# rushi-the-neural-arch/PyTorch-DistributedTraining

Hardware: AMD Instinct MI355X
Metric: tokens/sec GPT-2-1.3B FSDP (whole node) (higher is better)
Workload: dtype bf16; 1 GPU; model=gpt2-1.3b, global_batch=96, seq_len=1024, parallelism=fsdp1, micro_batch_per_gpu=96, params=1313722368, hip_graph=False, optimizer=fused AdamW + global-norm clip

## Files before the change

### csrc/kernels/gemm.hip

```cpp
#include "common.h"
#include "gelu.h"
#include "reduce.h"
#include <stdlib.h>
#include <type_traits>

using namespace pdt;

namespace {

typedef __bf16 bf16x8_t __attribute__((ext_vector_type(8)));
typedef short v4i16 __attribute__((ext_vector_type(4)));
typedef int v4i __attribute__((ext_vector_type(4)));
typedef __attribute__((address_space(3))) v4i16 lds_v4i16;
typedef __attribute__((address_space(3))) u16x8 lds_u16x8;
typedef __attribute__((address_space(3))) void lds_void;
typedef __attribute__((address_space(3))) const char lds_cchar;

constexpr int TM = 256, TN = 256, KB = 64, NTH = 256;
constexpr int OPB = TM * KB * 2;
constexpr int STB = 2 * OPB;
constexpr int PIECES = OPB / (NTH * 16);

enum { L_NT = 0, L_TT = 1 };
enum { E_PLAIN = 0, E_BIAS = 1, E_GELU = 2, E_DGELU = 3, E_F32 = 4 };
// ... 306 lines not shown
    if constexpr (EPI == E_DGELU) {
#pragma unroll
      for (int j = 0; j < 8; ++j)
#pragma unroll
        for (int r = 0; r < 4; ++r) {
          float v = cs[j][r];
          v += __shfl_xor(v, 1);
          v += __shfl_xor(v, 2);
          v += __shfl_xor(v, 4);
          v += __shfl_xor(v, 8);
          cs[j][r] = v;
        }
      __syncthreads();
      float* red = reinterpret_cast<float*>(smem);
      if ((lane & 15) == 0) {
#pragma unroll
        for (int j = 0; j < 8; ++j)
#pragma unroll
          for (int r = 0; r < 4; ++r) red[wr * 256 + 128 * wc + 16 * j + 4 * (lane >> 4) + r] = cs[j][r];
      }
      __syncthreads();
      p.ws[(int64_t)tm * p.N + n0 + tid] = red[tid] + red[256 + tid];
    }
  }
  }
}

}
#include "gemm_kloop.inc"
namespace {

constexpr int RING = 2 * STB;
constexpr int STAGE_BYTES = 32768;
constexpr int SMEM3 = RING + STAGE_BYTES;

template <int I, int N, class F>
__device__ __forceinline__ void sfor(F&& f) {
  if constexpr (I < N) {
    f(std::integral_constant<int, I>{});
    sfor<I + 1, N>(f);
  }
}

template <int K>
__device__ __forceinline__ f32x4 acc_tile() {
  float x, y, z, w;
  asm volatile("v_accvgpr_read_b32 %0, a%c4\n\tv_accvgpr_read_b32 %1, a%c5\n\t"
               "v_accvgpr_read_b32 %2, a%c6\n\tv_accvgpr_read_b32 %3, a%c7"
               : "=v"(x), "=v"(y), "=v"(z), "=v"(w)
               : "i"(4 * K), "i"(4 * K + 1), "i"(4 * K + 2), "i"(4 * K + 3));
  return f32x4{x, y, z, w};
}

__device__ __forceinline__ uint32_t stg_off(int q, int col) {
  return (uint32_t)(q * 512 + ((((col >> 3) ^ q) & 15) | ((col >> 3) & 16)) * 16 + (col & 7) * 2);
}
__device__ __forceinline__ int stg_row(int r, int q) { return 128 * (q >> 5) + 32 * r + (q & 31); }
__device__ __forceinline__ void stg_read(const char* img, u16x8 (&buf)[8], int w, int lane) {
#pragma unroll
  for (int it = 0; it < 8; ++it) {
    const int q = 16 * w + 2 * it + (lane >> 5), c16 = lane & 31;
    buf[it] = *reinterpret_cast<const u16x8*>(img + q * 512 + ((c16 ^ (q & 15)) & 15 | (c16 & 16)) * 16);
  }
}
typedef unsigned int u32x4 __attribute__((ext_vector_type(4)));
__device__ __forceinline__ __amdgpu_buffer_rsrc_t tile_rsrc(const bf16_t* base, int64_t ldc, int m0, int n0) {
  return __builtin_amdgcn_make_buffer_rsrc((void*)(base + (int64_t)m0 * ldc + n0), (short)0,
                                           (int)((255 * ldc + 256) * 2), 0x00020000);
}
__device__ __forceinline__ uint32_t stg_voff(int64_t ldc, int w, int lane) {
  return (uint32_t)(128 * (w >> 1) + 16 * (w & 1) + (lane >> 5)) * ((uint32_t)ldc * 2u) + (uint32_t)(lane & 31) * 16u;
}
__device__ __forceinline__ float row16_sum(float v) {
  v += __int_as_float(__builtin_amdgcn_update_dpp(0, __float_as_int(v), 0xB1, 0xF, 0xF, false));
  v += __int_as_float(__builtin_amdgcn_update_dpp(0, __float_as_int(v), 0x4E, 0xF, 0xF, false));
  v += __int_as_float(__builtin_amdgcn_update_dpp(0, __float_as_int(v), 0x141, 0xF, 0xF, false));
  v += __int_as_float(__builtin_amdgcn_update_dpp(0, __float_as_int(v), 0x140, 0xF, 0xF, false));
  return v;
}
__device__ __forceinline__ void stg_write_out(const u16x8 (&buf)[8], __amdgpu_buffer_rsrc_t rs, uint32_t vo,
                                              uint32_t ldc2, int r) {
#pragma unroll
  for (int it = 0; it < 8; ++it)
    __builtin_amdgcn_raw_buffer_store_b128(__builtin_bit_cast(u32x4, buf[it]), rs, (int)vo,
                                           (int)((32 * r + 2 * it) * ldc2), 0);
}
__device__ __forceinline__ void stg_fetch(u16x8 (&t)[8], __amdgpu_buffer_rsrc_t rs, uint32_t vo, uint32_t ldc2, int r) {
#pragma unroll
  for (int it = 0; it < 8; ++it)
    t[it] = __builtin_bit_cast(u16x8, __builtin_amdgcn_raw_buffer_load_b128(rs, (int)vo,
                                                                            (int)((32 * r + 2 * it) * ldc2), 0));
}
__device__ __forceinline__ void stg_put(char* img, const u16x8 (&t)[8], int w, int lane) {
#pragma unroll
  for (int it = 0; it < 8; ++it) {
    const int q = 16 * w + 2 * it + (lane >> 5), c16 = lane & 31;
    *reinterpret_cast<u16x8*>(img + q * 512 + ((c16 ^ (q & 15)) & 15 | (c16 & 16)) * 16) = t[it];
  }
}
__device__ __forceinline__ void stg_dma_round0(const bf16_t* src, int64_t ldc, int m0, int n0, uint32_t img_lds,
                                               int w, int lane) {
  const uint64_t base = (uint64_t)(uintptr_t)(src + (int64_t)m0 * ldc + n0);
  v4i rsrc;
  rsrc[0] = (int)(uint32_t)base;
  rsrc[1] = (int)((base >> 32) & 0xffff);
  rsrc[2] = (int)(uint32_t)((255 * ldc + 256) * 2);
  rsrc[3] = 0x00020000;
  const int hi = lane >> 5, p = lane & 31;
  const uint32_t row0 = (uint32_t)(128 * (w >> 1) + 16 * (w & 1));
  const uint32_t ldc2 = (uint32_t)ldc * 2u;
  uint32_t vo[8], so[8];
#pragma unroll
  for (int i = 0; i < 8; ++i) {
    const uint32_t c16 = (uint32_t)(((p ^ (2 * i + hi)) & 15) | (p & 16));
    vo[i] = (uint32_t)hi * ldc2 + c16 * 16u;
    so[i] = __builtin_amdgcn_readfirstlane((row0 + 2 * i) * ldc2);
  }
  const uint32_t m = __builtin_amdgcn_readfirstlane(img_lds + 16 * w * 512);
  asm volatile(
      "s_mov_b32 m0, %[m]\n\ts_nop 0\n\tbuffer_load_dwordx4 %[v0], %[rs], %[s0] offen lds\n\t"
      "s_add_u32 m0, m0, 1024\n\ts_nop 0\n\tbuffer_load_dwordx4 %[v1], %[rs], %[s1] offen lds\n\t"
      "s_add_u32 m0, m0, 1024\n\ts_nop 0\n\tbuffer_load_dwordx4 %[v2], %[rs], %[s2] offen lds\n\t"
      "s_add_u32 m0, m0, 1024\n\ts_nop 0\n\tbuffer_load_dwordx4 %[v3], %[rs], %[s3] offen lds\n\t"
      "s_add_u32 m0, m0, 1024\n\ts_nop 0\n\tbuffer_load_dwordx4 %[v4], %[rs], %[s4] offen lds\n\t"
      "s_add_u32 m0, m0, 1024\n\ts_nop 0\n\tbuffer_load_dwordx4 %[v5], %[rs], %[s5] offen lds\n\t"
      "s_add_u32 m0, m0, 1024\n\ts_nop 0\n\tbuffer_load_dwordx4 %[v6], %[rs], %[s6] offen lds\n\t"
      "s_add_u32 m0, m0, 1024\n\ts_nop 0\n\tbuffer_load_dwordx4 %[v7], %[rs], %[s7] offen lds"
      :
      : [m] "s"(m), [rs] "s"(rsrc), [v0] "v"(vo[0]), [v1] "v"(vo[1]), [v2] "v"(vo[2]), [v3] "v"(vo[3]),
        [v4] "v"(vo[4]), [v5] "v"(vo[5]), [v6] "v"(vo[6]), [v7] "v"(vo[7]), [s0] "s"(so[0]), [s1] "s"(so[1]),
        [s2] "s"(so[2]), [s3] "s"(so[3]), [s4] "s"(so[4]), [s5] "s"(so[5]), [s6] "s"(so[6]), [s7] "s"(so[7])
      : "memory", "scc");
}

__device__ __forceinline__ int item_tid(int wv) {
  int l;
  asm volatile("v_mbcnt_lo_u32_b32 %0, -1, 0\n\tv_mbcnt_hi_u32_b32 %0, -1, %0" : "=v"(l));
  return wv * 64 + l;
}
__device__ __forceinline__ int opaque_s(int x) {
  asm volatile("" : "+s"(x));
  return x;
}

__device__ __forceinline__ v4i scalar_rsrc(const void* base, uint32_t nbytes) {
  const uint64_t a = (uint64_t)(uintptr_t)base;
  v4i r;
  r[0] = (int)(uint32_t)a; r[1] = (int)((a >> 32) & 0xffff); r[2] = (int)nbytes; r[3] = 0x00020000;
  return r;
}
__device__ __forceinline__ void preload_bias(u16x4 (&b)[8], const bf16_t* bias, int n0, int lcol) {
  const v4i rs = scalar_rsrc(bias + n0, 512);
  const uint32_t vo = (uint32_t)lcol * 2u;
  asm volatile("buffer_load_dwordx2 %0, %8, %9, 0 offen offset:0\n\t"
               "buffer_load_dwordx2 %1, %8, %9, 0 offen offset:32\n\t"
               "buffer_load_dwordx2 %2, %8, %9, 0 offen offset:64\n\t"
               "buffer_load_dwordx2 %3, %8, %9, 0 offen offset:96\n\t"
               "buffer_load_dwordx2 %4, %8, %9, 0 offen offset:128\n\t"
               "buffer_load_dwordx2 %5, %8, %9, 0 offen offset:160\n\t"
               "buffer_load_dwordx2 %6, %8, %9, 0 offen offset:192\n\t"
               "buffer_load_dwordx2 %7, %8, %9, 0 offen offset:224"
               : "=&v"(b[0]), "=&v"(b[1]), "=&v"(b[2]), "=&v"(b[3]), "=&v"(b[4]), "=&v"(b[5]), "=&v"(b[6]),
                 "=&v"(b[7])
               : "v"(vo), "s"(rs)
               : "memory");
}
__device__ __forceinline__ void preload_round1(u16x8 (&t)[8], const bf16_t* src, int64_t ldc, int m0, int n0,
                                               uint32_t vo) {
  const v4i rs = scalar_rsrc(src + (int64_t)m0 * ldc + n0, (uint32_t)((255 * ldc + 256) * 2));
  const uint32_t l2 = (uint32_t)ldc * 2u;
  asm volatile("buffer_load_dwordx4 %0, %8, %9, %10 offen\n\t"
               "buffer_load_dwordx4 %1, %8, %9, %11 offen\n\t"
               "buffer_load_dwordx4 %2, %8, %9, %12 offen\n\t"
               "buffer_load_dwordx4 %3, %8, %9, %13 offen\n\t"
               "buffer_load_dwordx4 %4, %8, %9, %14 offen\n\t"
               "buffer_load_dwordx4 %5, %8, %9, %15 offen\n\t"
               "buffer_load_dwordx4 %6, %8, %9, %16 offen\n\t"
               "buffer_load_dwordx4 %7, %8, %9, %17 offen"
               : "=&v"(t[0]), "=&v"(t[1]), "=&v"(t[2]), "=&v"(t[3]), "=&v"(t[4]), "=&v"(t[5]), "=&v"(t[6]),
                 "=&v"(t[7])
               : "v"(vo), "s"(rs), "s"(32 * l2), "s"(34 * l2), "s"(36 * l2), "s"(38 * l2), "s"(40 * l2),
                 "s"(42 * l2), "s"(44 * l2), "s"(46 * l2)
               : "memory");
}
template <class V, int N>
__device__ __forceinline__ void settle(V (&x)[N]) {
#pragma unroll
  for (int i = 0; i < N; ++i) asm volatile("" : "+v"(x[i]));
}

template <int LAYOUT>
struct ItemOps {
  int tm, tn, m0, n0, split, T;
  uint32_t alo, ahi, blo, bhi;
  __device__ __forceinline__ void init(const GemmArgs& p, int item, int ntiles) {
    split = item / ntiles;
    tile_of(p, item - split * ntiles, ntiles, tm, tn);
    m0 = tm * TM; n0 = tn * TN;
    const int kbeg = split * p.k_per_split;
    T = min(p.K - kbeg, p.k_per_split) / KB;
    uint64_t a0, b0;
    if (LAYOUT == L_NT) {
      a0 = (uint64_t)(uintptr_t)p.A + ((uint64_t)m0 * p.lda + kbeg) * 2;
      b0 = (uint64_t)(uintptr_t)p.B + ((uint64_t)n0 * p.ldb + kbeg) * 2;
    } else {
      a0 = (uint64_t)(uintptr_t)p.A + ((uint64_t)kbeg * p.lda + m0) * 2;
      b0 = (uint64_t)(uintptr_t)p.B + ((uint64_t)kbeg * p.ldb + n0) * 2;
    }
    alo = (uint32_t)a0; ahi = (uint32_t)(a0 >> 32) & 0xffffu;
    blo = (uint32_t)b0; bhi = (uint32_t)(b0 >> 32) & 0xffffu;
  }
  __device__ __forceinline__ void skip2(uint64_t astep, uint64_t bstep) { skipn(2 * astep, 2 * bstep); }
  __device__ __forceinline__ void skip1(uint64_t astep, uint64_t bstep) { skipn(astep, bstep); }
  __device__ __forceinline__ void skipn(uint64_t da, uint64_t dbb) {
    const uint64_t a = (((uint64_t)ahi << 32) | alo) + da, b = (((uint64_t)bhi << 32) | blo) + dbb;
    alo = (uint32_t)a; ahi = (uint32_t)(a >> 32) & 0xffffu;
    blo = (uint32_t)b; bhi = (uint32_t)(b >> 32) & 0xffffu;
  }
};

__device__ __forceinline__ uint64_t stamp() {
  uint64_t t;
  asm volatile("s_memtime %0\n\ts_waitcnt lgkmcnt(0)" : "=s"(t) : : "memory");
  return t;
}

template <int LAYOUT, int EPI, int DIAG = 0, bool P3 = false>
__global__ __launch_bounds__(NTH, 1) void gemm_asm_kernel(GemmArgs p) {
  __shared__ __attribute__((aligned(16))) char smem[SMEM3];
  const uint32_t lds_addr = (uint32_t)(uintptr_t)(lds_void*)smem;
  const int tid = threadIdx.x, w = tid >> 6, lane = tid & 63;
  const int wr = w >> 1, wc = w & 1;
  const int wv = __builtin_amdgcn_readfirstlane(w);
  const int ntiles = (p.M / TM) * (p.N / TN);
  const int splits = (p.K + p.k_per_split - 1) / p.k_per_split;
  const int nall = ntiles * splits;

  uint64_t astep, bstep;
  uint32_t abytes, bbytes, rsa, rsb;
  int32_t db;
  if (LAYOUT == L_NT) {
    astep = bstep = KB * 2;
    abytes = (uint32_t)((TM - 1) * p.lda * 2 + KB * 2);
    bbytes = (uint32_t)((TN - 1) * p.ldb * 2 + KB * 2);
    rsa = (uint32_t)(32 * p.lda * 2);
    rsb = (uint32_t)(32 * p.ldb * 2);
    db = OPB + 16384 * (wc - wr);
  } else {
    astep = (uint64_t)KB * p.lda * 2;
    bstep = (uint64_t)KB * p.ldb * 2;
    abytes = (uint32_t)((KB - 1) * p.lda * 2 + TM * 2);
    bbytes = (uint32_t)((KB - 1) * p.ldb * 2 + TN * 2);
    rsa = (uint32_t)(8 * p.lda * 2);
    rsb = (uint32_t)(8 * p.ldb * 2);
    db = OPB + 256 * (wc - wr);
  }
  auto lane_ops = [&](int t, uint32_t& voa0, uint32_t& voa1, uint32_t& vob0, uint32_t& vob1, uint32_t& rd0,
                      uint32_t& rd1) {
    const int lw = t >> 6, ll = t & 63, lwr = lw >> 1;
    if (LAYOUT == L_NT) {
      const int row = 8 * lw + (ll >> 3);
      const int c = (ll & 7) ^ ((row >> 1) & 7);
      voa0 = voa1 = (uint32_t)(row * p.lda * 2 + c * 16);
      vob0 = vob1 = (uint32_t)(row * p.ldb * 2 + c * 16);
      const int x = ll & 15, g = ll >> 4, h = (x >> 1) & 7;
      rd0 = lds_addr + 16384 * lwr + (uint32_t)(x * 128 + 16 * (g ^ h));
      rd1 = lds_addr + 16384 * lwr + (uint32_t)(x * 128 + 16 * ((4 + g) ^ h));
    } else {
      const int r0 = 2 * lw + (ll >> 5);
      voa0 = (uint32_t)(r0 * p.lda * 2 + ((ll & 31) ^ tt_f(r0)) * 16);
      voa1 = (uint32_t)(r0 * p.lda * 2 + ((ll & 31) ^ tt_f(r0 + 8)) * 16);
      vob0 = (uint32_t)(r0 * p.ldb * 2 + ((ll & 31) ^ tt_f(r0)) * 16);
      vob1 = (uint32_t)(r0 * p.ldb * 2 + ((ll & 31) ^ tt_f(r0 + 8)) * 16);
      const int g = ll >> 4, q = (ll >> 2) & 3, pp = ll & 3;
      rd0 = lds_addr + 256 * lwr + (uint32_t)((8 * g + q) * 512 + 16 * (pp >> 1) + 8 * (pp & 1));
      rd1 = (uint32_t)tt_f(8 * g + q);
    }
  };
  const uint32_t m0b = __builtin_amdgcn_readfirstlane(lds_addr + w * 1024);
  const int dbs = __builtin_amdgcn_readfirstlane(db);
  const uint32_t asl = (uint32_t)astep, ash = (uint32_t)(astep >> 32);
  const uint32_t bsl = (uint32_t)bstep, bsh = (uint32_t)(bstep >> 32);
  constexpr int NST = EPI == E_F32 ? 64 : EPI == E_GELU ? 64 + 8 : EPI == E_DGELU ? 32 + 1 + 8 + 8 : EPI == E_BIAS ? 40 : 32;
  constexpr int WNX = 16 + NST < 63 ? 16 + NST : 63;
  char* const img = smem + RING;

#define PDT_KLOOP_CLOBBERS                                                                                      \
  "memory", "scc", "s80", "s81", "s82", "s83", "s84", "s85", "s86", "s87", "s88", "s89", "s90", "s91",         \
  "v64", "v65", "v66", "v67", "v68", "v69", "v70", "v71", "v72", "v73", "v74", "v75", "v76", "v77", "v78",     \
  "v79", "v80", "v81", "v82", "v83", "v84", "v85", "v86", "v87", "v88", "v89", "v90", "v91", "v92", "v93",     \
  "v94", "v95", "v128", "v129", "v130", "v131", "v132", "v133", "v134", "v135", "v136", "v137", "v138", "v139", \
  "v140", "v141", "v142", "v143", "v144", "v145", "v146", "v147", "v148", "v149", "v150", "v151", "v152",      \
  "v153", "v154", "v155", "v156", "v157", "v158", "v159", "v160", "v161", "v162", "v163", "v164", "v165",      \
  "v166", "v167", "v168", "v169", "v170", "v171", "v172", "v173", "v174", "v175", "v176", "v177", "v178",      \
  "v179", "v180", "v181", "v182", "v183", "v184", "v185", "v186", "v187", "v188", "v189", "v190", "v191",      \
  "v192", "v193", "v194", "v195", "v196", "v197", "v198", "v199", "v200", "v201", "v202", "v203", "v204",      \
  "v205", "v206", "v207", "v208", "v209", "v210", "v211", "v212", "v213", "v214", "v215", "v216", "v217",      \
  "v218", "v219", "v220", "v221", "v222", "v223", "v224", "v225", "v226", "v227", "v228", "v229", "v230",      \
  "v231", "v232", "v233", "v234", "v235", "v236", "v237", "v238", "v239", "v240", "v241", "v242", "v243",      \
  "v244", "v245", "v246", "v247", "v248", "v249", "v250", "v251", "v252", "v253", "v254", "v255",              \
  PDT_AGPR_CLOBBERS
#define PDT_ITEM_OPS                                                                                            \
  [alo] "s"(lo.alo), [ahi] "s"(lo.ahi), [anr] "s"(abytes), [blo] "s"(lo.blo), [bhi] "s"(lo.bhi),               \
      [bnr] "s"(bbytes), [m0b] "s"(m0b), [rsa] "s"(rsa), [rsb] "s"(rsb), [asl] "s"(asl), [ash] "s"(ash),         \
      [bsl] "s"(bsl), [bsh] "s"(bsh), [cnt] "s"(cnt), [first] "s"(first), [wnx] "i"(WNX), [hnx] "s"(hnx),        \
      [nalo] "s"(nxt.alo), [nahi] "s"(nxt.ahi), [nblo] "s"(nxt.blo), [nbhi] "s"(nxt.bhi), [db] "s"(dbs)
#define PDT_KLOOP_NT_ASM(MAC)                                                                                     \
  asm volatile(MAC : : PDT_ITEM_OPS, [voa] "v"(voa0), [vob] "v"(vob0), [rd0] "v"(rd0), [rd1] "v"(rd1)           \
               : PDT_KLOOP_CLOBBERS)
#define PDT_KLOOP_TT_ASM(MAC)                                                                                     \
  asm volatile(MAC : : PDT_ITEM_OPS, [voa0] "v"(voa0), [voa1] "v"(voa1), [vob0] "v"(vob0), [vob1] "v"(vob1),    \
               [rd0] "v"(rd0), [rdx] "v"(rd1) : PDT_KLOOP_CLOBBERS)
#define PDT_KLOOP_NT_ASM3(MAC)                                                                                    \
  asm volatile(MAC : : PDT_ITEM_OPS, [voa] "v"(voa0), [vob] "v"(vob0), [rd0] "v"(rd0), [rd1] "v"(rd1)           \
               : PDT_KLOOP_CLOBBERS, "v96", "v97")
#define PDT_KLOOP_TT_ASM3(MAC)                                                                                    \
  asm volatile(MAC : : PDT_ITEM_OPS, [voa0] "v"(voa0), [voa1] "v"(voa1), [vob0] "v"(vob0), [vob1] "v"(vob1),    \
               [rd0] "v"(rd0), [rdx] "v"(rd1)                                                                    \
               : PDT_KLOOP_CLOBBERS, "v96", "v97", "v98", "v99", "v100", "v101", "v102", "v103")
#define PDT_STAMP_OUTS                                                                                            \
  [st0] "=s"(ph[0]), [st1] "=s"(ph[1]), [st2] "=s"(ph[2]), [st3] "=s"(ph[3]), [st4] "=s"(ph[4]),               \
      [st5] "=s"(ph[5]), [st6] "=s"(ph[6]), [st7] "=s"(ph[7])
#define PDT_KLOOP_NT_ASM_ST(MAC)                                                                                  \
  asm volatile(MAC : PDT_STAMP_OUTS : PDT_ITEM_OPS, [voa] "v"(voa0), [vob] "v"(vob0), [rd0] "v"(rd0),            \
               [rd1] "v"(rd1) : PDT_KLOOP_CLOBBERS, "s92", "s93", "s94", "s95", "s96", "s97", "s98", "s99")
#define PDT_KLOOP_TT_ASM_ST(MAC)                                                                                  \
  asm volatile(MAC : PDT_STAMP_OUTS : PDT_ITEM_OPS, [voa0] "v"(voa0), [voa1] "v"(voa1), [vob0] "v"(vob0),         \
               [vob1] "v"(vob1), [rd0] "v"(rd0), [rdx] "v"(rd1)                                                  \
               : PDT_KLOOP_CLOBBERS, "s92", "s93", "s94", "s95", "s96", "s97", "s98", "s99")

  ItemOps<LAYOUT> cur;
  int item = blockIdx.x;
  cur.init(p, item, ntiles);
  int first = 1;
  while (true) {
    const int next_item = item + (int)gridDim.x;
    const bool has_next = next_item < nall;
    ItemOps<LAYOUT> nxt = cur;
    if (has_next) {
      GemmArgs q = p;
      q.M = opaque_s(p.M); q.N = opaque_s(p.N); q.xpr = opaque_s(p.xpr); q.grp = opaque_s(p.grp);
      q.K = opaque_s(p.K); q.k_per_split = opaque_s(p.k_per_split);
      nxt.init(q, next_item, opaque_s(ntiles));
    }
    const int hnx = P3 ? 0 : __builtin_amdgcn_readfirstlane((((nall - 1 - next_item) >> 31) + 1) & ~cur.T & 1);
    const int cnt = __builtin_amdgcn_readfirstlane(cur.T);
    first = __builtin_amdgcn_readfirstlane(first);
    ItemOps<LAYOUT> lo = cur;
    if (!first) lo.skip2(astep, bstep);
    lo.alo = __builtin_amdgcn_readfirstlane(lo.alo); lo.ahi = __builtin_amdgcn_readfirstlane(lo.ahi);
    lo.blo = __builtin_amdgcn_readfirstlane(lo.blo); lo.bhi = __builtin_amdgcn_readfirstlane(lo.bhi);
    uint64_t st0 = 0, st1 = 0, rt0 = 0;
    if (DIAG) { st0 = stamp(); rt0 = __builtin_amdgcn_s_memrealtime(); }
    const int ltid = item_tid(wv);
    uint32_t voa0, voa1, vob0, vob1, rd0, rd1;
    lane_ops(ltid, voa0, voa1, vob0, vob1, rd0, rd1);
    u16x4 pb[8];
    u16x8 pa[8];
    if constexpr (EPI == E_DGELU) {
      stg_dma_round0(p.aux, p.ldc, cur.m0, cur.n0, lds_addr + RING, ltid >> 6, ltid & 63);
      preload_round1(pa, p.aux, p.ldc, cur.m0, cur.n0, stg_voff(p.ldc, ltid >> 6, ltid & 63));
    }
    if constexpr (EPI == E_BIAS || EPI == E_GELU) preload_bias(pb, p.bias, cur.n0, 128 * ((ltid >> 6) & 1) + 4 * ((ltid & 63) >> 4));
    uint32_t ph[8] = {0, 0, 0, 0, 0, 0, 0, 0};
    if constexpr (DIAG) {
      if constexpr (LAYOUT == L_NT) PDT_KLOOP_NT_ASM_ST(PDT_GEMM_KLOOP_NT_STAMPS);
      else PDT_KLOOP_TT_ASM_ST(PDT_GEMM_KLOOP_TT_STAMPS);
    } else if constexpr (P3) {
      if constexpr (LAYOUT == L_NT) PDT_KLOOP_NT_ASM3(PDT_GEMM_KLOOP_NT3);
      else PDT_KLOOP_TT_ASM3(PDT_GEMM_KLOOP_TT3);
    } else {
      if constexpr (LAYOUT == L_NT) PDT_KLOOP_NT_ASM(PDT_GEMM_KLOOP_NT);
      else PDT_KLOOP_TT_ASM(PDT_GEMM_KLOOP_TT);
    }
    if constexpr (EPI == E_DGELU) settle(pa);
    if constexpr (EPI == E_BIAS || EPI == E_GELU) settle(pb);
    if (DIAG) st1 = stamp();
    const int m0 = cur.m0, n0 = cur.n0, tm = cur.tm;

    const int etid = item_tid(wv);
    {
    const int tid = etid, w = etid >> 6, lane = etid & 63, wr = w >> 1, wc = w & 1;
    const int lrow = 128 * wr + (lane & 15);
    const int lcol = 128 * wc + 4 * (lane >> 4);
    if constexpr (EPI == E_F32) {
      float* C = p.ws + (int64_t)cur.split * p.M * p.N;
      sfor<0, 64>([&](auto kc) {
        constexpr int k = decltype(kc)::value;
        const f32x4 v = acc_tile<k>();
        *reinterpret_cast<f32x4*>(C + (int64_t)(m0 + lrow + 16 * (k >> 3)) * p.N + n0 + lcol + 16 * (k & 7)) = v;
      });
    } else {
      bf16_t* C = reinterpret_cast<bf16_t*>(p.C);
      u16x8 buf[8];
      float bj[8][4];
      if constexpr (EPI == E_BIAS || EPI == E_GELU) {
#pragma unroll
        for (int j = 0; j < 8; ++j)
#pragma unroll
          for (int r = 0; r < 4; ++r) bj[j][r] = bf2f(pb[j][r]);
      }
      float cs[8][4];
#pragma unroll
      for (int j = 0; j < 8; ++j)
#pragma unroll
        for (int r = 0; r < 4; ++r) cs[j][r] = 0.f;
      u16x8 aux[2][8];
      const uint32_t svo = stg_voff(p.ldc, w, lane), ldc2 = (uint32_t)(p.ldc * 2);
      const __amdgpu_buffer_rsrc_t rsc = tile_rsrc(C, p.ldc, m0, n0);
      if constexpr (EPI == E_DGELU) {
#pragma unroll
        for (int it = 0; it < 8; ++it) aux[1][it] = pa[it];
      }
      sfor<0, 4>([&](auto rc) {
        constexpr int r = decltype(rc)::value;
        if constexpr (EPI == E_DGELU && r > 0) {
          __syncthreads();
          stg_put(img, aux[r & 1], w, lane);
          if constexpr (r < 3) stg_fetch(aux[(r + 1) & 1], tile_rsrc(p.aux, p.ldc, m0, n0), svo, ldc2, r + 1);
        }
        __syncthreads();
        u16x4 dk[16];
        u16x4 hk[8];
        sfor<0, 16>([&](auto kc) {
          constexpr int kk = decltype(kc)::value, k = 16 * r + kk, i = k >> 3, j = k & 7;
          if constexpr (EPI == E_DGELU && (kk & 7) == 0) {
            sfor<0, 8>([&](auto hc) {
              constexpr int k2 = k + decltype(hc)::value, i2 = k2 >> 3, j2 = k2 & 7;
              hk[decltype(hc)::value] = *reinterpret_cast<const u16x4*>(
                  img + stg_off(32 * wr + 16 * (i2 & 1) + (lane & 15), lcol + 16 * j2));
            });
          }
          const f32x4 v = acc_tile<k>();
          const uint32_t at = stg_off(32 * wr + 16 * (i & 1) + (lane & 15), lcol + 16 * j);
          u16x4 o;
          if constexpr (EPI == E_DGELU) {
            const u16x4 hh = hk[kk & 7];
#pragma unroll
            for (int e = 0; e < 4; ++e) {
              const bf16_t gb = f2bf(v[e] * bf2f(hh[e]));
              o[e] = gb;
              cs[j][e] += bf2f(gb);
            }
          } else if constexpr (EPI == E_GELU) {
#pragma unroll
            for (int e = 0; e < 4; e += 2) {
              gelu_f32x2 y2, d2;
              gelu_fwd_grad2(gelu_f32x2{bf2f(f2bf(v[e] + bj[j][e])), bf2f(f2bf(v[e + 1] + bj[j][e + 1]))}, y2, d2);
              o[e] = f2bf(y2[0]); o[e + 1] = f2bf(y2[1]);
              dk[kk][e] = f2bf(d2[0]); dk[kk][e + 1] = f2bf(d2[1]);
            }
          } else {
#pragma unroll
            for (int e = 0; e < 4; ++e) o[e] = f2bf(EPI == E_BIAS ? v[e] + bj[j][e] : v[e]);
          }
          *reinterpret_cast<u16x4*>(img + at) = o;
        });
        __syncthreads();
        stg_read(img, buf, w, lane);
        stg_write_out(buf, rsc, svo, ldc2, r);
        if constexpr (EPI == E_GELU) {
          __syncthreads();
          sfor<0, 16>([&](auto kc) {
            constexpr int kk = decltype(kc)::value, k = 16 * r + kk, i = k >> 3, j = k & 7;
            const uint32_t at = stg_off(32 * wr + 16 * (i & 1) + (lane & 15), lcol + 16 * j);
            *reinterpret_cast<u16x4*>(img + at) = dk[kk];
          });
          __syncthreads();
          stg_read(img, buf, w, lane);
          stg_write_out(buf, tile_rsrc(p.aux_out, p.ldc, m0, n0), svo, ldc2, r);
        }
      });
      if constexpr (EPI == E_DGELU) {
#pragma unroll
        for (int j = 0; j < 8; ++j)
#pragma unroll
          for (int e = 0; e < 4; ++e) cs[j][e] = row16_sum(cs[j][e]);
        __syncthreads();
        float* red = reinterpret_cast<float*>(img);
        if ((lane & 15) == 0) {
#pragma unroll
          for (int j = 0; j < 8; ++j)
#pragma unroll
            for (int e = 0; e < 4; ++e) red[wr * 256 + lcol + 16 * j + e] = cs[j][e];
        }
        __syncthreads();
        p.ws[(int64_t)tm * p.N + n0 + tid] = red[tid] + red[256 + tid];
      }
      __syncthreads();
    }
    }
    if (DIAG) {
      const uint64_t st2 = stamp();
      if (tid == 0) {
        uint64_t* d = reinterpret_cast<uint64_t*>(p.ws) + 8 * (int64_t)item;
        d[0] = st0; d[1] = st1; d[2] = st2; d[3] = rt0;
        for (int i = 0; i < 4; ++i) d[4 + i] = ((uint64_t)ph[2 * i + 1] << 32) | ph[2 * i];
      }
    }
    if (!has_next) break;
    item = next_item;
    first = 1 - hnx;
    cur = nxt;
  }
#undef PDT_KLOOP_CLOBBERS
#undef PDT_ITEM_OPS
#undef PDT_KLOOP_NT_ASM3
#undef PDT_KLOOP_TT_ASM3
#undef PDT_KLOOP_NT_ASM_ST
#undef PDT_KLOOP_TT_ASM_ST
#undef PDT_STAMP_OUTS
#undef PDT_KLOOP_NT_ASM
#undef PDT_KLOOP_TT_ASM
}

static int persist_grid(int nitems) {
  static const int cus = [] {
    int dev = 0, n = 0;
    if (hipGetDevice(&dev) != hipSuccess || hipDeviceGetAttribute(&n, hipDeviceAttributeMultiprocessorCount, dev) !=
                                                hipSuccess)
      n = 256;
    return n;
  }();
  int g = cus < nitems ? cus : nitems;
  return g >= 8 ? g & ~7 : g;
}

bool use_p3(int layout, const GemmArgs& a, int items, int grid) {
  static const int forced = [] { const char* e = getenv("PDT_GEMM_P3"); return e ? atoi(e) : -1; }();
  const int T = a.k_per_split / KB;
  if (T < 6 || forced == 0) return false;
  if (forced == 1) return true;
  const int cb = a.xpr > 0 ? (a.N / TN) / (8 / a.xpr) : a.N / TN;
  return layout == L_TT ? (items > grid && (a.M / TM) * (a.N / TN) < grid) : (a.k_per_split >= 8192 || cb <= 8);
}

template <int LAYOUT>
int launch_asm_layout(int epi, const GemmArgs& a, int splits, hipStream_t s) {
  const int items = (a.M / TM) * (a.N / TN) * splits;
  const dim3 grid(persist_grid(items), 1);
  if (use_p3(LAYOUT, a, items, (int)grid.x) && (epi == E_PLAIN || epi == E_BIAS || epi == E_F32)) {
    switch (epi) {
      case E_PLAIN: gemm_asm_kernel<LAYOUT, E_PLAIN, 0, true><<<grid, NTH, 0, s>>>(a); break;
      case E_BIAS: gemm_asm_kernel<LAYOUT, E_BIAS, 0, true><<<grid, NTH, 0, s>>>(a); break;
      default: gemm_asm_kernel<LAYOUT, E_F32, 0, true><<<grid, NTH, 0, s>>>(a); break;
    }
    return (int)hipGetLastError();
  }
  switch (epi) {
    case E_PLAIN: gemm_asm_kernel<LAYOUT, E_PLAIN><<<grid, NTH, 0, s>>>(a); break;
// ... 96 lines not shown
    gemm_splitk_reduce_kernel<<<grid_for(n4, 256, 256 * 16), 256, 0, s>>>(ws, (bf16_t*)C, n4, splits, M * N);
    if (ldc != N) return (int)hipErrorInvalidValue;
  }
  if (epi == E_DGELU)
    red::col_reduce<bf16_t>(ws, (int)(M / TM), (int)N, (bf16_t*)dbias, ws + (M / TM) * N, 0, s);
  return (int)hipGetLastError();
}

PDT_API int pdt_gemm2_bf16(int layout, int epi, const void* A, const void* B, void* C, int64_t M, int64_t N,
                           int64_t K, int64_t lda, int64_t ldb, int64_t ldc, const void* bias, const void* aux,
                           void* aux_out, void* dbias, float* ws, int splits, hipStream_t s) {
  if (!pdt_gemm_ok(layout, M, N, K, lda, ldb, splits) || ldc < N || ldc % 8) return (int)hipErrorInvalidValue;
  if (K / splits < 2 * KB) return (int)hipErrorInvalidValue;
  if (epi < 0 || epi > E_DGELU) return (int)hipErrorInvalidValue;
  if (splits > 1 && (epi != E_PLAIN || !ws)) return (int)hipErrorInvalidValue;
  if ((epi == E_BIAS || epi == E_GELU) && !bias) return (int)hipErrorInvalidValue;
  if (epi == E_GELU && !aux_out) return (int)hipErrorInvalidValue;
  if (epi == E_DGELU && (!aux || !ws || !dbias)) return (int)hipErrorInvalidValue;
  GemmArgs a{};
  a.A = (const bf16_t*)A; a.B = (const bf16_t*)B; a.C = C;
  a.bias = (const bf16_t*)bias; a.aux = (const bf16_t*)aux; a.aux_out = (bf16_t*)aux_out; a.ws = ws;
  a.M = (int)M; a.N = (int)N; a.K = (int)K; a.lda = lda; a.ldb = ldb; a.ldc = ldc;
  a.k_per_split = (int)(K / splits);
  a.xpr = xcd_cut((int)(M / TM), (int)(N / TN));
  a.grp = xcd_grp((int)(M / TM), (int)(N / TN), (int)(K / splits), a.xpr);
  const int run_epi = splits > 1 ? E_F32 : epi;
  if (splits > 1) a.ldc = N;
  int err = layout == L_NT ? launch_asm_layout<L_NT>(run_epi, a, splits, s)
                           : launch_asm_layout<L_TT>(run_epi, a, splits, s);
  if (err) return err;
  if (splits > 1) {
    if (ldc != N) return (int)hipErrorInvalidValue;
    const int64_t n4 = M * N / 4;
    gemm_splitk_reduce_kernel<<<grid_for(n4, 256, 256 * 16), 256, 0, s>>>(ws, (bf16_t*)C, n4, splits, M * N);
  }
  if (epi == E_DGELU)
    red::col_reduce<bf16_t>(ws, (int)(M / TM), (int)N, (bf16_t*)dbias, ws + (M / TM) * N, 0, s);
  return (int)hipGetLastError();
}

PDT_API int pdt_gemm_stamps_epi_bf16(int layout, int epi, const void* A, const void* B, void* C, int64_t M, int64_t N,
                                     int64_t K, int64_t lda, int64_t ldb, const void* bias, void* aux_out,
                                     void* stamps, hipStream_t s);
PDT_API int pdt_gemm_stamps_bf16(int layout, const void* A, const void* B, void* C, int64_t M, int64_t N, int64_t K,
                                 int64_t lda, int64_t ldb, void* stamps, hipStream_t s) {
  if (!pdt_gemm_ok(layout, M, N, K, lda, ldb, 1) || K < 2 * KB || !stamps) return (int)hipErrorInvalidValue;
  return pdt_gemm_stamps_epi_bf16(layout, E_PLAIN, A, B, C, M, N, K, lda, ldb, nullptr, nullptr, stamps, s);
}

PDT_API int pdt_gemm_stamps_epi_bf16(int layout, int epi, const void* A, const void* B, void* C, int64_t M, int64_t N,
                                     int64_t K, int64_t lda, int64_t ldb, const void* bias, void* aux_out,
                                     void* stamps, hipStream_t s) {
  if (!pdt_gemm_ok(layout, M, N, K, lda, ldb, 1) || K < 2 * KB || !stamps) return (int)hipErrorInvalidValue;
  if (epi != E_PLAIN && (layout != L_NT || !bias || (epi == E_GELU && !aux_out) || (epi != E_BIAS && epi != E_GELU)))
    return (int)hipErrorInvalidValue;
  GemmArgs a{};
  a.A = (const bf16_t*)A; a.B = (const bf16_t*)B; a.C = C; a.ws = (float*)stamps;
  a.bias = (const bf16_t*)bias; a.aux_out = (bf16_t*)aux_out;
  a.M = (int)M; a.N = (int)N; a.K = (int)K; a.lda = lda; a.ldb = ldb; a.ldc = N; a.k_per_split = (int)K;
  a.xpr = xcd_cut((int)(M / TM), (int)(N / TN));
  a.grp = xcd_grp((int)(M / TM), (int)(N / TN), (int)K, a.xpr);
  const dim3 grid(persist_grid((int)((M / TM) * (N / TN))), 1);
  if (layout == L_TT) gemm_asm_kernel<L_TT, E_PLAIN, 1><<<grid, NTH, 0, s>>>(a);
  else if (epi == E_BIAS) gemm_asm_kernel<L_NT, E_BIAS, 1><<<grid, NTH, 0, s>>>(a);
  else if (epi == E_GELU) gemm_asm_kernel<L_NT, E_GELU, 1><<<grid, NTH, 0, s>>>(a);
  else gemm_asm_kernel<L_NT, E_PLAIN, 1><<<grid, NTH, 0, s>>>(a);
  return (int)hipGetLastError();
}
```

Baseline: 151,000 tokens/s.

## Restructure GEMM epilogue into double-buffered half-tile units with nontemporal stores

```diff
diff --git a/csrc/kernels/gemm.hip b/csrc/kernels/gemm.hip
--- a/csrc/kernels/gemm.hip
+++ b/csrc/kernels/gemm.hip
@@ -382,15 +382,16 @@
   return f32x4{x, y, z, w};
 }
 
+constexpr int HALF = STAGE_BYTES / 2;
 __device__ __forceinline__ uint32_t stg_off(int q, int col) {
   return (uint32_t)(q * 512 + ((((col >> 3) ^ q) & 15) | ((col >> 3) & 16)) * 16 + (col & 7) * 2);
 }
-__device__ __forceinline__ int stg_row(int r, int q) { return 128 * (q >> 5) + 32 * r + (q & 31); }
-__device__ __forceinline__ void stg_read(const char* img, u16x8 (&buf)[8], int w, int lane) {
-#pragma unroll
-  for (int it = 0; it < 8; ++it) {
-    const int q = 16 * w + 2 * it + (lane >> 5), c16 = lane & 31;
-    buf[it] = *reinterpret_cast<const u16x8*>(img + q * 512 + ((c16 ^ (q & 15)) & 15 | (c16 & 16)) * 16);
+__device__ __forceinline__ int stg_row(int i, int q) { return 128 * (q >> 4) + 16 * i + (q & 15); }
+__device__ __forceinline__ void stg_read(const char* half, u16x8 (&buf)[4], int w, int lane) {
+#pragma unroll
+  for (int it = 0; it < 4; ++it) {
+    const int q = 8 * w + 2 * it + (lane >> 5), c16 = lane & 31;
+    buf[it] = *reinterpret_cast<const u16x8*>(half + q * 512 + ((c16 ^ (q & 15)) & 15 | (c16 & 16)) * 16);
   }
 }
 typedef unsigned int u32x4 __attribute__((ext_vector_type(4)));
@@ -399,7 +400,7 @@
                                            (int)((255 * ldc + 256) * 2), 0x00020000);
 }
 __device__ __forceinline__ uint32_t stg_voff(int64_t ldc, int w, int lane) {
-  return (uint32_t)(128 * (w >> 1) + 16 * (w & 1) + (lane >> 5)) * ((uint32_t)ldc * 2u) + (uint32_t)(lane & 31) * 16u;
+  return (uint32_t)(128 * (w >> 1) + 8 * (w & 1) + (lane >> 5)) * ((uint32_t)ldc * 2u) + (uint32_t)(lane & 31) * 16u;
 }
 __device__ __forceinline__ float row16_sum(float v) {
   v += __int_as_float(__builtin_amdgcn_update_dpp(0, __float_as_int(v), 0xB1, 0xF, 0xF, false));
@@ -408,28 +409,43 @@
   v += __int_as_float(__builtin_amdgcn_update_dpp(0, __float_as_int(v), 0x140, 0xF, 0xF, false));
   return v;
 }
-__device__ __forceinline__ void stg_write_out(const u16x8 (&buf)[8], __amdgpu_buffer_rsrc_t rs, uint32_t vo,
-                                              uint32_t ldc2, int r) {
-#pragma unroll
-  for (int it = 0; it < 8; ++it)
+#ifndef PDT_GEMM_NT
+#define PDT_GEMM_NT 7
+#endif
+constexpr int POL_AUX_OUT = (PDT_GEMM_NT & 1) ? 2 : 0, POL_C_ACT = (PDT_GEMM_NT & 2) ? 2 : 0,
+              POL_AUX_IN = (PDT_GEMM_NT & 4) ? 2 : 0, POL_C_LIN = (PDT_GEMM_NT & 8) ? 2 : 0;
+#if PDT_GEMM_NT & 4
+#define PDT_AUX_LD_NT " nt"
+#else
+#define PDT_AUX_LD_NT ""
+#endif
+template <int POL>
+__device__ __forceinline__ void stg_write_out(const u16x8 (&buf)[4], __amdgpu_buffer_rsrc_t rs, uint32_t vo,
+                                              uint32_t ldc2, int i) {
+  __builtin_amdgcn_sched_barrier(0);
+#pragma unroll
+  for (int it = 0; it < 4; ++it)
     __builtin_amdgcn_raw_buffer_store_b128(__builtin_bit_cast(u32x4, buf[it]), rs, (int)vo,
-                                           (int)((32 * r + 2 * it) * ldc2), 0);
-}
-__device__ __forceinline__ void stg_fetch(u16x8 (&t)[8], __amdgpu_buffer_rsrc_t rs, uint32_t vo, uint32_t ldc2, int r) {
-#pragma unroll
-  for (int it = 0; it < 8; ++it)
+                                           (int)((16 * i + 2 * it) * ldc2), POL);
+  __builtin_amdgcn_sched_barrier(0);
+  asm volatile("s_nop 3");
+  __builtin_amdgcn_sched_barrier(0);
+}
+__device__ __forceinline__ void stg_fetch(u16x8 (&t)[4], __amdgpu_buffer_rsrc_t rs, uint32_t vo, uint32_t ldc2, int i) {
+#pragma unroll
+  for (int it = 0; it < 4; ++it)
     t[it] = __builtin_bit_cast(u16x8, __builtin_amdgcn_raw_buffer_load_b128(rs, (int)vo,
-                                                                            (int)((32 * r + 2 * it) * ldc2), 0));
-}
-__device__ __forceinline__ void stg_put(char* img, const u16x8 (&t)[8], int w, int lane) {
-#pragma unroll
-  for (int it = 0; it < 8; ++it) {
-    const int q = 16 * w + 2 * it + (lane >> 5), c16 = lane & 31;
-    *reinterpret_cast<u16x8*>(img + q * 512 + ((c16 ^ (q & 15)) & 15 | (c16 & 16)) * 16) = t[it];
-  }
-}
-__device__ __forceinline__ void stg_dma_round0(const bf16_t* src, int64_t ldc, int m0, int n0, uint32_t img_lds,
-                                               int w, int lane) {
+                                                                            (int)((16 * i + 2 * it) * ldc2), POL_AUX_IN));
+}
+__device__ __forceinline__ void stg_put(char* half, const u16x8 (&t)[4], int w, int lane) {
+#pragma unroll
+  for (int it = 0; it < 4; ++it) {
+    const int q = 8 * w + 2 * it + (lane >> 5), c16 = lane & 31;
+    *reinterpret_cast<u16x8*>(half + q * 512 + ((c16 ^ (q & 15)) & 15 | (c16 & 16)) * 16) = t[it];
+  }
+}
+__device__ __forceinline__ void stg_dma_unit0(const bf16_t* src, int64_t ldc, int m0, int n0, uint32_t img_lds,
+                                              int w, int lane) {
   const uint64_t base = (uint64_t)(uintptr_t)(src + (int64_t)m0 * ldc + n0);
   v4i rsrc;
   rsrc[0] = (int)(uint32_t)base;
@@ -437,29 +453,24 @@
   rsrc[2] = (int)(uint32_t)((255 * ldc + 256) * 2);
   rsrc[3] = 0x00020000;
   const int hi = lane >> 5, p = lane & 31;
-  const uint32_t row0 = (uint32_t)(128 * (w >> 1) + 16 * (w & 1));
+  const uint32_t row0 = (uint32_t)(128 * (w >> 1) + 8 * (w & 1));
   const uint32_t ldc2 = (uint32_t)ldc * 2u;
-  uint32_t vo[8], so[8];
-#pragma unroll
-  for (int i = 0; i < 8; ++i) {
-    const uint32_t c16 = (uint32_t)(((p ^ (2 * i + hi)) & 15) | (p & 16));
+  uint32_t vo[4], so[4];
+#pragma unroll
+  for (int i = 0; i < 4; ++i) {
+    const uint32_t c16 = (uint32_t)(((p ^ (8 * (w & 1) + 2 * i + hi)) & 15) | (p & 16));
     vo[i] = (uint32_t)hi * ldc2 + c16 * 16u;
     so[i] = __builtin_amdgcn_readfirstlane((row0 + 2 * i) * ldc2);
   }
-  const uint32_t m = __builtin_amdgcn_readfirstlane(img_lds + 16 * w * 512);
+  const uint32_t m = __builtin_amdgcn_readfirstlane(img_lds + 8 * w * 512);
   asm volatile(
-      "s_mov_b32 m0, %[m]\n\ts_nop 0\n\tbuffer_load_dwordx4 %[v0], %[rs], %[s0] offen lds\n\t"
-      "s_add_u32 m0, m0, 1024\n\ts_nop 0\n\tbuffer_load_dwordx4 %[v1], %[rs], %[s1] offen lds\n\t"
-      "s_add_u32 m0, m0, 1024\n\ts_nop 0\n\tbuffer_load_dwordx4 %[v2], %[rs], %[s2] offen lds\n\t"
-      "s_add_u32 m0, m0, 1024\n\ts_nop 0\n\tbuffer_load_dwordx4 %[v3], %[rs], %[s3] offen lds\n\t"
-      "s_add_u32 m0, m0, 1024\n\ts_nop 0\n\tbuffer_load_dwordx4 %[v4], %[rs], %[s4] offen lds\n\t"
-      "s_add_u32 m0, m0, 1024\n\ts_nop 0\n\tbuffer_load_dwordx4 %[v5], %[rs], %[s5] offen lds\n\t"
-      "s_add_u32 m0, m0, 1024\n\ts_nop 0\n\tbuffer_load_dwordx4 %[v6], %[rs], %[s6] offen lds\n\t"
-      "s_add_u32 m0, m0, 1024\n\ts_nop 0\n\tbuffer_load_dwordx4 %[v7], %[rs], %[s7] offen lds"
+      "s_mov_b32 m0, %[m]\n\ts_nop 0\n\tbuffer_load_dwordx4 %[v0], %[rs], %[s0] offen" PDT_AUX_LD_NT " lds" "\n\t"
+      "s_add_u32 m0, m0, 1024\n\ts_nop 0\n\tbuffer_load_dwordx4 %[v1], %[rs], %[s1] offen" PDT_AUX_LD_NT " lds" "\n\t"
+      "s_add_u32 m0, m0, 1024\n\ts_nop 0\n\tbuffer_load_dwordx4 %[v2], %[rs], %[s2] offen" PDT_AUX_LD_NT " lds" "\n\t"
+      "s_add_u32 m0, m0, 1024\n\ts_nop 0\n\tbuffer_load_dwordx4 %[v3], %[rs], %[s3] offen" PDT_AUX_LD_NT " lds"
       :
       : [m] "s"(m), [rs] "s"(rsrc), [v0] "v"(vo[0]), [v1] "v"(vo[1]), [v2] "v"(vo[2]), [v3] "v"(vo[3]),
-        [v4] "v"(vo[4]), [v5] "v"(vo[5]), [v6] "v"(vo[6]), [v7] "v"(vo[7]), [s0] "s"(so[0]), [s1] "s"(so[1]),
-        [s2] "s"(so[2]), [s3] "s"(so[3]), [s4] "s"(so[4]), [s5] "s"(so[5]), [s6] "s"(so[6]), [s7] "s"(so[7])
+        [s0] "s"(so[0]), [s1] "s"(so[1]), [s2] "s"(so[2]), [s3] "s"(so[3])
       : "memory", "scc");
 }
 
@@ -495,22 +506,22 @@
                : "v"(vo), "s"(rs)
                : "memory");
 }
-__device__ __forceinline__ void preload_round1(u16x8 (&t)[8], const bf16_t* src, int64_t ldc, int m0, int n0,
-                                               uint32_t vo) {
+__device__ __forceinline__ void preload_units12(u16x8 (&t)[2][4], const bf16_t* src, int64_t ldc, int m0, int n0,
+                                                uint32_t vo) {
   const v4i rs = scalar_rsrc(src + (int64_t)m0 * ldc + n0, (uint32_t)((255 * ldc + 256) * 2));
   const uint32_t l2 = (uint32_t)ldc * 2u;
-  asm volatile("buffer_load_dwordx4 %0, %8, %9, %10 offen\n\t"
-               "buffer_load_dwordx4 %1, %8, %9, %11 offen\n\t"
-               "buffer_load_dwordx4 %2, %8, %9, %12 offen\n\t"
-               "buffer_load_dwordx4 %3, %8, %9, %13 offen\n\t"
-               "buffer_load_dwordx4 %4, %8, %9, %14 offen\n\t"
-               "buffer_load_dwordx4 %5, %8, %9, %15 offen\n\t"
-               "buffer_load_dwordx4 %6, %8, %9, %16 offen\n\t"
-               "buffer_load_dwordx4 %7, %8, %9, %17 offen"
-               : "=&v"(t[0]), "=&v"(t[1]), "=&v"(t[2]), "=&v"(t[3]), "=&v"(t[4]), "=&v"(t[5]), "=&v"(t[6]),
-                 "=&v"(t[7])
-               : "v"(vo), "s"(rs), "s"(32 * l2), "s"(34 * l2), "s"(36 * l2), "s"(38 * l2), "s"(40 * l2),
-                 "s"(42 * l2), "s"(44 * l2), "s"(46 * l2)
+  asm volatile("buffer_load_dwordx4 %0, %8, %9, %10 offen" PDT_AUX_LD_NT "\n\t"
+               "buffer_load_dwordx4 %1, %8, %9, %11 offen" PDT_AUX_LD_NT "\n\t"
+               "buffer_load_dwordx4 %2, %8, %9, %12 offen" PDT_AUX_LD_NT "\n\t"
+               "buffer_load_dwordx4 %3, %8, %9, %13 offen" PDT_AUX_LD_NT "\n\t"
+               "buffer_load_dwordx4 %4, %8, %9, %14 offen" PDT_AUX_LD_NT "\n\t"
+               "buffer_load_dwordx4 %5, %8, %9, %15 offen" PDT_AUX_LD_NT "\n\t"
+               "buffer_load_dwordx4 %6, %8, %9, %16 offen" PDT_AUX_LD_NT "\n\t"
+               "buffer_load_dwordx4 %7, %8, %9, %17 offen" PDT_AUX_LD_NT
+               : "=&v"(t[1][0]), "=&v"(t[1][1]), "=&v"(t[1][2]), "=&v"(t[1][3]), "=&v"(t[0][0]), "=&v"(t[0][1]),
+                 "=&v"(t[0][2]), "=&v"(t[0][3])
+               : "v"(vo), "s"(rs), "s"(16 * l2), "s"(18 * l2), "s"(20 * l2), "s"(22 * l2), "s"(32 * l2),
+                 "s"(34 * l2), "s"(36 * l2), "s"(38 * l2)
                : "memory");
 }
 template <class V, int N>
@@ -549,6 +560,7 @@
   }
 };
 
+constexpr int STAMP_SLOTS = 32;
 __device__ __forceinline__ uint64_t stamp() {
   uint64_t t;
   asm volatile("s_memtime %0\n\ts_waitcnt lgkmcnt(0)" : "=s"(t) : : "memory");
@@ -611,7 +623,7 @@
   const int dbs = __builtin_amdgcn_readfirstlane(db);
   const uint32_t asl = (uint32_t)astep, ash = (uint32_t)(astep >> 32);
   const uint32_t bsl = (uint32_t)bstep, bsh = (uint32_t)(bstep >> 32);
-  constexpr int NST = EPI == E_F32 ? 64 : EPI == E_GELU ? 64 + 8 : EPI == E_DGELU ? 32 + 1 + 8 + 8 : EPI == E_BIAS ? 40 : 32;
+  constexpr int NST = EPI == E_F32 ? 64 : EPI == E_GELU ? 64 + 8 : EPI == E_DGELU ? 32 + 20 + 1 + 4 + 8 : EPI == E_BIAS ? 40 : 32;
   constexpr int WNX = 16 + NST < 63 ? 16 + NST : 63;
   char* const img = smem + RING;
 
@@ -681,15 +693,16 @@
     lo.alo = __builtin_amdgcn_readfirstlane(lo.alo); lo.ahi = __builtin_amdgcn_readfirstlane(lo.ahi);
     lo.blo = __builtin_amdgcn_readfirstlane(lo.blo); lo.bhi = __builtin_amdgcn_readfirstlane(lo.bhi);
     uint64_t st0 = 0, st1 = 0, rt0 = 0;
+    uint64_t us[17] = {};
     if (DIAG) { st0 = stamp(); rt0 = __builtin_amdgcn_s_memrealtime(); }
     const int ltid = item_tid(wv);
     uint32_t voa0, voa1, vob0, vob1, rd0, rd1;
     lane_ops(ltid, voa0, voa1, vob0, vob1, rd0, rd1);
     u16x4 pb[8];
-    u16x8 pa[8];
+    u16x8 pa[2][4];
     if constexpr (EPI == E_DGELU) {
-      stg_dma_round0(p.aux, p.ldc, cur.m0, cur.n0, lds_addr + RING, ltid >> 6, ltid & 63);
-      preload_round1(pa, p.aux, p.ldc, cur.m0, cur.n0, stg_voff(p.ldc, ltid >> 6, ltid & 63));
+      stg_dma_unit0(p.aux, p.ldc, cur.m0, cur.n0, lds_addr + RING, ltid >> 6, ltid & 63);
+      preload_units12(pa, p.aux, p.ldc, cur.m0, cur.n0, stg_voff(p.ldc, ltid >> 6, ltid & 63));
     }
     if constexpr (EPI == E_BIAS || EPI == E_GELU) preload_bias(pb, p.bias, cur.n0, 128 * ((ltid >> 6) & 1) + 4 * ((ltid & 63) >> 4));
     uint32_t ph[8] = {0, 0, 0, 0, 0, 0, 0, 0};
@@ -703,7 +716,7 @@
       if constexpr (LAYOUT == L_NT) PDT_KLOOP_NT_ASM(PDT_GEMM_KLOOP_NT);
       else PDT_KLOOP_TT_ASM(PDT_GEMM_KLOOP_TT);
     }
-    if constexpr (EPI == E_DGELU) settle(pa);
+    if constexpr (EPI == E_DGELU) { settle(pa[0]); settle(pa[1]); }
     if constexpr (EPI == E_BIAS || EPI == E_GELU) settle(pb);
     if (DIAG) st1 = stamp();
     const int m0 = cur.m0, n0 = cur.n0, tm = cur.tm;
@@ -722,7 +735,7 @@
       });
     } else {
       bf16_t* C = reinterpret_cast<bf16_t*>(p.C);
-      u16x8 buf[8];
+      u16x8 buf[4];
       float bj[8][4];
       if constexpr (EPI == E_BIAS || EPI == E_GELU) {
 #pragma unroll
@@ -735,79 +748,97 @@
       for (int j = 0; j < 8; ++j)
 #pragma unroll
         for (int r = 0; r < 4; ++r) cs[j][r] = 0.f;
-      u16x8 aux[2][8];
       const uint32_t svo = stg_voff(p.ldc, w, lane), ldc2 = (uint32_t)(p.ldc * 2);
       const __amdgpu_buffer_rsrc_t rsc = tile_rsrc(C, p.ldc, m0, n0);
-      if constexpr (EPI == E_DGELU) {
-#pragma unroll
-        for (int it = 0; it < 8; ++it) aux[1][it] = pa[it];
-      }
-      sfor<0, 4>([&](auto rc) {
-        constexpr int r = decltype(rc)::value;
-        if constexpr (EPI == E_DGELU && r > 0) {
-          __syncthreads();
-          stg_put(img, aux[r & 1], w, lane);
-          if constexpr (r < 3) stg_fetch(aux[(r + 1) & 1], tile_rsrc(p.aux, p.ldc, m0, n0), svo, ldc2, r + 1);
-        }
-        __syncthreads();
-        u16x4 dk[16];
-        u16x4 hk[8];
-        sfor<0, 16>([&](auto kc) {
-          constexpr int kk = decltype(kc)::value, k = 16 * r + kk, i = k >> 3, j = k & 7;
-          if constexpr (EPI == E_DGELU && (kk & 7) == 0) {
-            sfor<0, 8>([&](auto hc) {
-              constexpr int k2 = k + decltype(hc)::value, i2 = k2 >> 3, j2 = k2 & 7;
-              hk[decltype(hc)::value] = *reinterpret_cast<const u16x4*>(
-                  img + stg_off(32 * wr + 16 * (i2 & 1) + (lane & 15), lcol + 16 * j2));
-            });
-          }
-          const f32x4 v = acc_tile<k>();
-          const uint32_t at = stg_off(32 * wr + 16 * (i & 1) + (lane & 15), lcol + 16 * j);
-          u16x4 o;
-          if constexpr (EPI == E_DGELU) {
-            const u16x4 hh = hk[kk & 7];
-#pragma unroll
-            for (int e = 0; e < 4; ++e) {
-              const bf16_t gb = f2bf(v[e] * bf2f(hh[e]));
-              o[e] = gb;
-              cs[j][e] += bf2f(gb);
-            }
-          } else if constexpr (EPI == E_GELU) {
+      constexpr int PC = (EPI == E_GELU || EPI == E_DGELU) ? POL_C_ACT : POL_C_LIN;
+      char* const h0 = img;
+      char* const h1 = img + HALF;
+      const int qrow = 16 * wr + (lane & 15);
+      __syncthreads();
+      if constexpr (DIAG) us[0] = stamp();
+      if constexpr (EPI == E_GELU) {
+        const __amdgpu_buffer_rsrc_t rsx = tile_rsrc(p.aux_out, p.ldc, m0, n0);
+        sfor<0, 8>([&](auto ic) {
+          constexpr int i = decltype(ic)::value;
+          if constexpr (i > 0) stg_read(h1, buf, w, lane);
+          u16x4 dk[8];
+          sfor<0, 8>([&](auto jc) {
+            constexpr int j = decltype(jc)::value;
+            const f32x4 v = acc_tile<8 * i + j>();
+            u16x4 o;
 #pragma unroll
             for (int e = 0; e < 4; e += 2) {
               gelu_f32x2 y2, d2;
               gelu_fwd_grad2(gelu_f32x2{bf2f(f2bf(v[e] + bj[j][e])), bf2f(f2bf(v[e + 1] + bj[j][e + 1]))}, y2, d2);
               o[e] = f2bf(y2[0]); o[e + 1] = f2bf(y2[1]);
-              dk[kk][e] = f2bf(d2[0]); dk[kk][e + 1] = f2bf(d2[1]);
+              dk[j][e] = f2bf(d2[0]); dk[j][e + 1] = f2bf(d2[1]);
             }
-          } else {
-#pragma unroll
-            for (int e = 0; e < 4; ++e) o[e] = f2bf(EPI == E_BIAS ? v[e] + bj[j][e] : v[e]);
+            *reinterpret_cast<u16x4*>(h0 + stg_off(qrow, lcol + 16 * j)) = o;
+          });
+          if constexpr (i > 0) stg_write_out<POL_AUX_OUT>(buf, rsx, svo, ldc2, i - 1);
+          __syncthreads();
+          if constexpr (DIAG) us[2 * i + 1] = stamp();
+          stg_read(h0, buf, w, lane);
+          sfor<0, 8>([&](auto jc) {
+            constexpr int j = decltype(jc)::value;
+            *reinterpret_cast<u16x4*>(h1 + stg_off(qrow, lcol + 16 * j)) = dk[j];
+          });
+          stg_write_out<PC>(buf, rsc, svo, ldc2, i);
+          __syncthreads();
+          if constexpr (DIAG) us[2 * i + 2] = stamp();
+        });
+        stg_read(h1, buf, w, lane);
+        stg_write_out<POL_AUX_OUT>(buf, rsx, svo, ldc2, 7);
+      } else {
+        u16x8 aux[2][4];
+        if constexpr (EPI == E_DGELU) {
+#pragma unroll
+          for (int it = 0; it < 4; ++it) { aux[0][it] = pa[0][it]; aux[1][it] = pa[1][it]; }
+        }
+        sfor<0, 8>([&](auto uc) {
+          constexpr int u = decltype(uc)::value;
+          char* const X = (u & 1) ? h1 : h0;
+          char* const Y = (u & 1) ? h0 : h1;
+          if constexpr (u > 0) stg_read(Y, buf, w, lane);
+          u16x4 hk[8];
+          if constexpr (EPI == E_DGELU) {
+            sfor<0, 8>([&](auto jc) {
+              constexpr int j = decltype(jc)::value;
+              hk[j] = *reinterpret_cast<const u16x4*>(X + stg_off(qrow, lcol + 16 * j));
+            });
+            if constexpr (u < 7) stg_put(Y, aux[(u + 1) & 1], w, lane);
+            if constexpr (u + 3 < 8) stg_fetch(aux[(u + 1) & 1], tile_rsrc(p.aux, p.ldc, m0, n0), svo, ldc2, u + 3);
           }
-          *reinterpret_cast<u16x4*>(img + at) = o;
+          sfor<0, 8>([&](auto jc) {
+            constexpr int j = decltype(jc)::value;
+            const f32x4 v = acc_tile<8 * u + j>();
+            u16x4 o;
+            if constexpr (EPI == E_DGELU) {
+#pragma unroll
+              for (int e = 0; e < 4; ++e) {
+                const bf16_t gb = f2bf(v[e] * bf2f(hk[j][e]));
+                o[e] = gb;
+                cs[j][e] += bf2f(gb);
+              }
+            } else {
+#pragma unroll
+              for (int e = 0; e < 4; ++e) o[e] = f2bf(EPI == E_BIAS ? v[e] + bj[j][e] : v[e]);
+            }
+            *reinterpret_cast<u16x4*>(X + stg_off(qrow, lcol + 16 * j)) = o;
+          });
+          if constexpr (u > 0) stg_write_out<PC>(buf, rsc, svo, ldc2, u - 1);
+          __syncthreads();
+          if constexpr (DIAG) us[u + 1] = stamp();
         });
-        __syncthreads();
-        stg_read(img, buf, w, lane);
-        stg_write_out(buf, rsc, svo, ldc2, r);
-        if constexpr (EPI == E_GELU) {
-          __syncthreads();
-          sfor<0, 16>([&](auto kc) {
-            constexpr int kk = decltype(kc)::value, k = 16 * r + kk, i = k >> 3, j = k & 7;
-            const uint32_t at = stg_off(32 * wr + 16 * (i & 1) + (lane & 15), lcol + 16 * j);
-            *reinterpret_cast<u16x4*>(img + at) = dk[kk];
-          });
-          __syncthreads();
-          stg_read(img, buf, w, lane);
-          stg_write_out(buf, tile_rsrc(p.aux_out, p.ldc, m0, n0), svo, ldc2, r);
-        }
-      });
+        stg_read(h1, buf, w, lane);
+        stg_write_out<PC>(buf, rsc, svo, ldc2, 7);
+      }
       if constexpr (EPI == E_DGELU) {
 #pragma unroll
         for (int j = 0; j < 8; ++j)
 #pragma unroll
           for (int e = 0; e < 4; ++e) cs[j][e] = row16_sum(cs[j][e]);
-        __syncthreads();
-        float* red = reinterpret_cast<float*>(img);
+        float* red = reinterpret_cast<float*>(h0);
         if ((lane & 15) == 0) {
 #pragma unroll
           for (int j = 0; j < 8; ++j)
@@ -815,7 +846,8 @@
             for (int e = 0; e < 4; ++e) red[wr * 256 + lcol + 16 * j + e] = cs[j][e];
         }
         __syncthreads();
-        p.ws[(int64_t)tm * p.N + n0 + tid] = red[tid] + red[256 + tid];
+        float* colp = DIAG ? reinterpret_cast<float*>(p.aux_out) : p.ws;
+        colp[(int64_t)tm * p.N + n0 + tid] = red[tid] + red[256 + tid];
       }
       __syncthreads();
     }
@@ -823,9 +855,11 @@
     if (DIAG) {
       const uint64_t st2 = stamp();
       if (tid == 0) {
-        uint64_t* d = reinterpret_cast<uint64_t*>(p.ws) + 8 * (int64_t)item;
+        uint64_t* d = reinterpret_cast<uint64_t*>(p.ws) + STAMP_SLOTS * (int64_t)item;
         d[0] = st0; d[1] = st1; d[2] = st2; d[3] = rt0;
         for (int i = 0; i < 4; ++i) d[4 + i] = ((uint64_t)ph[2 * i + 1] << 32) | ph[2 * i];
+#pragma unroll
+        for (int i = 0; i < 17; ++i) d[8 + i] = us[i];
       }
     }
     if (!has_next) break;
@@ -1028,11 +1062,12 @@
                                      int64_t K, int64_t lda, int64_t ldb, const void* bias, void* aux_out,
                                      void* stamps, hipStream_t s) {
   if (!pdt_gemm_ok(layout, M, N, K, lda, ldb, 1) || K < 2 * KB || !stamps) return (int)hipErrorInvalidValue;
-  if (epi != E_PLAIN && (layout != L_NT || !bias || (epi == E_GELU && !aux_out) || (epi != E_BIAS && epi != E_GELU)))
+  if (epi != E_PLAIN && (layout != L_NT || !bias || (epi != E_BIAS && !aux_out) || epi < E_BIAS || epi > E_DGELU))
     return (int)hipErrorInvalidValue;
   GemmArgs a{};
   a.A = (const bf16_t*)A; a.B = (const bf16_t*)B; a.C = C; a.ws = (float*)stamps;
   a.bias = (const bf16_t*)bias; a.aux_out = (bf16_t*)aux_out;
+  if (epi == E_DGELU) { a.aux = (const bf16_t*)bias; a.bias = nullptr; }
   a.M = (int)M; a.N = (int)N; a.K = (int)K; a.lda = lda; a.ldb = ldb; a.ldc = N; a.k_per_split = (int)K;
   a.xpr = xcd_cut((int)(M / TM), (int)(N / TN));
   a.grp = xcd_grp((int)(M / TM), (int)(N / TN), (int)K, a.xpr);
@@ -1040,6 +1075,7 @@
   if (layout == L_TT) gemm_asm_kernel<L_TT, E_PLAIN, 1><<<grid, NTH, 0, s>>>(a);
   else if (epi == E_BIAS) gemm_asm_kernel<L_NT, E_BIAS, 1><<<grid, NTH, 0, s>>>(a);
   else if (epi == E_GELU) gemm_asm_kernel<L_NT, E_GELU, 1><<<grid, NTH, 0, s>>>(a);
+  else if (epi == E_DGELU) gemm_asm_kernel<L_NT, E_DGELU, 1><<<grid, NTH, 0, s>>>(a);
   else gemm_asm_kernel<L_NT, E_PLAIN, 1><<<grid, NTH, 0, s>>>(a);
   return (int)hipGetLastError();
 }
```

Result: no change. 151,300 tokens/s (median of 5 runs) (+0.2%).
